# zjkang/Relation-DETR

Hardware: AMD Instinct MI355X
Metric: images/sec @ 800×1333, 300 queries, R50 4-level; achieved HBM GB/s (higher is better)
Workload: dtype bf16; 1 GPU; relation_detr_resnet50_800_1333 transformer stack from feature pyramids: 6 encoder layers (MSDA self-attn, S=22323, 4 levels) + two-stage top-k + 6 decoder layers (relation-biased self-attn + MSDA cross-attn + box refinement) + top-300 detections; backbone/neck excluded; batch_per_gpu=4, global_batch=4, queries=900, levels=4, launch=hipGraph replay, streams=2, gemm_tuning=False, parallelism=image-parallel x1

## Files before the change

### relation_detr_amd/csrc/linear.hip

```cpp
#include <cstdlib>

#include "launch.h"

namespace rdetr {

typedef __bf16 ln_bf16x8 __attribute__((ext_vector_type(8)));

constexpr int kLinK = 256;
constexpr int kLinThreads = 512;
constexpr int kLinRows = 32;

template <int NT, bool RELU>
__global__ __launch_bounds__(kLinThreads) void linear_k256_kernel(const uint16_t *__restrict__ x, long long ldx,
                                                                  const uint16_t *__restrict__ w, const uint16_t *__restrict__ bias,
                                                                  long long M, int N, uint16_t *__restrict__ out, long long ldo, int dbg,
                                                                  const unsigned char *__restrict__ row_mask, int hm_S)
{
    extern __shared__ __attribute__((aligned(16))) unsigned char lin_lds[];
    u32x4 *wl = reinterpret_cast<u32x4 *>(lin_lds);
    float *bl = reinterpret_cast<float *>(lin_lds + NT * 8 * 64 * 16);
    const int tid = threadIdx.x, lane = tid & 63, wave = tid >> 6;
    const int col = lane & 15, g = lane >> 4;
    const int n0 = blockIdx.y * (NT * 16);

    {
        constexpr int kPer = NT * 16 * 32 / kLinThreads;
        u32x4 piece[kPer];
#pragma unroll
        for (int i = 0; i < kPer; ++i) {
            const int idx = i * kLinThreads + tid, c = idx >> 5, p = idx & 31;
            piece[i] = n0 + c < N ? *reinterpret_cast<const u32x4 *>(w + (size_t)(n0 + c) * kLinK + 8 * p) : u32x4{0u, 0u, 0u, 0u};
        }
#pragma unroll
        for (int i = 0; i < kPer; ++i) {
            const int idx = i * kLinThreads + tid, c = idx >> 5, p = idx & 31;
            const int t = 2 * (c >> 5) + ((c >> 2) & 1), m = 4 * ((c >> 3) & 3) + (c & 3);
            wl[(t * 8 + (p >> 2)) * 64 + 16 * (p & 3) + m] = piece[i];
        }
    }
    for (int i = tid; i < NT * 16; i += kLinThreads) bl[i] = (bias && n0 + i < N) ? bf16_bits_to_f32(bias[n0 + i]) : 0.f;
    __syncthreads();

    const long long nsteps = (M + kLinRows - 1) / kLinRows;
    constexpr int kWaves = kLinThreads / 64;
    const long long stride = (long long)gridDim.x * kWaves;
    long long step = (long long)blockIdx.x * kWaves + wave;

    u32x4 xc[2][8], xn[2][8];
    auto load_rows = [&](long long st, u32x4 (&dst)[2][8]) {
#pragma unroll
        for (int cb = 0; cb < 2; ++cb) {
            const long long row = st * kLinRows + cb * 16 + col;
            const uint16_t *p = x + row * ldx + 8 * g;
#pragma unroll
            for (int s = 0; s < 8; ++s)
                dst[cb][s] = (st < nsteps && row < M) ? *reinterpret_cast<const u32x4 *>(p + 32 * s) : u32x4{0u, 0u, 0u, 0u};
        }
    };
    load_rows(step, xc);
    for (; step < nsteps; step += stride) {
        load_rows(step + stride, xn);
        const long long row_a = step * kLinRows + col, row_b = row_a + 16;
        uint16_t *oa = out + row_a * ldo + n0 + 8 * g, *ob = out + row_b * ldo + n0 + 8 * g;
        bool zero_a = false, zero_b = false;
        if (hm_S) {
            const unsigned ia = (unsigned)row_a / (unsigned)hm_S, ib = (unsigned)row_b / (unsigned)hm_S;
            oa = out + ((long long)ia * 8 * hm_S + (row_a - (long long)ia * hm_S)) * 32 + 8 * g;
            ob = out + ((long long)ib * 8 * hm_S + (row_b - (long long)ib * hm_S)) * 32 + 8 * g;
            if (row_mask) {
                zero_a = row_a < M && row_mask[row_a] != 0;
                zero_b = row_b < M && row_mask[row_b] != 0;
            }
        }
#pragma unroll
        for (int u = 0; u < NT / 2; ++u) {
            f32x4 acc[2][2];
#pragma unroll
            for (int e = 0; e < 2; ++e) {
                const f32x4 b4 = *reinterpret_cast<const f32x4 *>(bl + 32 * u + 8 * g + 4 * e);
                acc[e][0] = b4;
                acc[e][1] = b4;
            }
            if (!(dbg & 2))
#pragma unroll
            for (int s = 0; s < 8; ++s) {
#pragma unroll
                for (int e = 0; e < 2; ++e) {
                    const ln_bf16x8 a = __builtin_bit_cast(ln_bf16x8, wl[((2 * u + e) * 8 + s) * 64 + lane]);
                    acc[e][0] = __builtin_amdgcn_mfma_f32_16x16x32_bf16(a, __builtin_bit_cast(ln_bf16x8, xc[0][s]), acc[e][0], 0, 0, 0);
                    acc[e][1] = __builtin_amdgcn_mfma_f32_16x16x32_bf16(a, __builtin_bit_cast(ln_bf16x8, xc[1][s]), acc[e][1], 0, 0, 0);
                }
            }
            if (n0 + 32 * u + 8 * g < N) {
#pragma unroll
                for (int cb = 0; cb < 2; ++cb) {
                    f32x4 lo = acc[0][cb], hi = acc[1][cb];
                    if (RELU) {
                        lo.x = fmaxf(lo.x, 0.f); lo.y = fmaxf(lo.y, 0.f); lo.z = fmaxf(lo.z, 0.f); lo.w = fmaxf(lo.w, 0.f);
                        hi.x = fmaxf(hi.x, 0.f); hi.y = fmaxf(hi.y, 0.f); hi.z = fmaxf(hi.z, 0.f); hi.w = fmaxf(hi.w, 0.f);
                    }
                    u32x4 pk;
                    pk.x = f32_to_bf16_bits(lo.x) | (f32_to_bf16_bits(lo.y) << 16);
                    pk.y = f32_to_bf16_bits(lo.z) | (f32_to_bf16_bits(lo.w) << 16);
                    pk.z = f32_to_bf16_bits(hi.x) | (f32_to_bf16_bits(hi.y) << 16);
                    pk.w = f32_to_bf16_bits(hi.z) | (f32_to_bf16_bits(hi.w) << 16);
                    if ((cb ? zero_b : zero_a)) pk = u32x4{0u, 0u, 0u, 0u};
                    const long long col_off = hm_S ? (long long)u * hm_S * 32 : 32 * u;
                    if ((cb ? row_b : row_a) < M && !((dbg & 1) && pk.x != 0x12345u)) *reinterpret_cast<u32x4 *>((cb ? ob : oa) + col_off) = pk;
                }
            }
            __builtin_amdgcn_sched_barrier(0);
        }
#pragma unroll
        for (int cb = 0; cb < 2; ++cb)
#pragma unroll
            for (int s = 0; s < 8; ++s) xc[cb][s] = xn[cb][s];
    }
}

template <int NT, bool RELU>
static int linear_launch(const uint16_t *x, long long ldx, const uint16_t *w, const uint16_t *bias, long long M, int N,
                         uint16_t *out, long long ldo, int chunks, hipStream_t st, const unsigned char *row_mask = nullptr, int hm_S = 0)
{
    constexpr int lds = NT * 8 * 64 * 16 + NT * 16 * 4;
    if (const int s = ensure_dynamic_lds<linear_k256_kernel<NT, RELU>>(lds)) return s;
    const long long steps = (M + kLinRows - 1) / kLinRows;
    long long gx = (steps + kLinThreads / 64 - 1) / (kLinThreads / 64);
    const long long cap = kCus / chunks > 0 ? kCus / chunks : 1;
    if (gx > cap) gx = cap;
    hipLaunchKernelGGL((linear_k256_kernel<NT, RELU>), dim3((unsigned)gx, (unsigned)chunks), dim3(kLinThreads), (size_t)lds, st, x, ldx, w, bias, M, N, out,
                       ldo, 0, row_mask, hm_S);
    return launch_status();
}


constexpr int kLnlThreads = 512;
constexpr int kLnlWaves = kLnlThreads / 64;

__global__ __launch_bounds__(256) void linear_pack_kernel(const uint16_t *__restrict__ w, u32x4 *__restrict__ packed)
{
    const int idx = blockIdx.x * 256 + threadIdx.x;
    if (idx >= 16 * 8 * 64) return;
    const int t = idx >> 9, s = (idx >> 6) & 7, l = idx & 63, m = l & 15, kb = l >> 4;
    const int n = 32 * (t >> 1) + 8 * (m >> 2) + 4 * (t & 1) + (m & 3);
    packed[idx] = *reinterpret_cast<const u32x4 *>(w + (size_t)n * kLinK + 32 * s + 8 * kb);
}

__global__ __launch_bounds__(kLnlThreads) void linear_ln_k256_kernel(const uint16_t *__restrict__ x, long long ldx,
                                                                     const uint16_t *__restrict__ packed,
                                                                     const uint16_t *__restrict__ bias,
                                                                     const uint16_t *__restrict__ res, long long ldr,
                                                                     const uint16_t *__restrict__ gamma,
                                                                     const uint16_t *__restrict__ beta, float eps, long long M,
                                                                     uint16_t *__restrict__ out, long long ldo)
{
    extern __shared__ __attribute__((aligned(16))) unsigned char lin_lds[];
    const u32x4 *wl = reinterpret_cast<const u32x4 *>(lin_lds);
    float *bl = reinterpret_cast<float *>(lin_lds + 16 * 8 * 64 * 16);
    const int tid = threadIdx.x, lane = tid & 63, wave = __builtin_amdgcn_readfirstlane(tid >> 6);
    const int col = lane & 15, g = lane >> 4;
    {
        const unsigned lane_off = (unsigned)lane * 16u;
#pragma unroll 1
        for (int i = 0; i < 128 / kLnlWaves; ++i) {
            const int f = wave * (128 / kLnlWaves) + i;
            const unsigned m0v = (unsigned)f * 1024u;
            const unsigned char *src = reinterpret_cast<const unsigned char *>(packed) + f * 1024;
            asm volatile("s_mov_b32 m0, %0\n\ts_nop 0\n\tglobal_load_lds_dwordx4 %1, %2" : : "s"(m0v), "v"(lane_off), "s"(src) : "memory", "m0");
        }
    }
    if (tid < 256) {
        bl[tid] = bias ? bf16_bits_to_f32(bias[tid]) : 0.f;
        bl[256 + tid] = bf16_bits_to_f32(gamma[tid]);
        bl[512 + tid] = bf16_bits_to_f32(beta[tid]);
    }
    const long long nsteps = (M + kLinRows - 1) / kLinRows;
    long long step = (long long)blockIdx.x * kLnlWaves + wave;
    const long long stride = (long long)gridDim.x * kLnlWaves;
    asm volatile("s_waitcnt vmcnt(0)" ::: "memory");
    __syncthreads();
    for (; step < nsteps; step += stride) {
        const long long row_a = step * kLinRows + col, row_b = row_a + 16;
        u32x4 xc[2][8];
#pragma unroll
        for (int s = 0; s < 8; ++s) {
            xc[0][s] = row_a < M ? *reinterpret_cast<const u32x4 *>(x + row_a * ldx + 32 * s + 8 * g) : u32x4{0u, 0u, 0u, 0u};
            xc[1][s] = row_b < M ? *reinterpret_cast<const u32x4 *>(x + row_b * ldx + 32 * s + 8 * g) : u32x4{0u, 0u, 0u, 0u};
        }
        f32x4 acc[16][2];
        {
            auto frag = [&](int i) -> u32x4 { return wl[((i & 15) * 8 + (i >> 4)) * 64 + lane]; };
            const f32x4 zero4 = {0.f, 0.f, 0.f, 0.f};
            u32x4 ring[3];
            ring[0] = frag(0);
            ring[1] = frag(1);
#pragma unroll
            for (int i = 0; i < 128; ++i) {
                if (i + 2 < 128) ring[(i + 2) % 3] = frag(i + 2);
                __builtin_amdgcn_sched_barrier(0);
                const int s = i >> 4, t = i & 15;
                const ln_bf16x8 a = __builtin_bit_cast(ln_bf16x8, ring[i % 3]);
                acc[t][0] = __builtin_amdgcn_mfma_f32_16x16x32_bf16(a, __builtin_bit_cast(ln_bf16x8, xc[0][s]), s ? acc[t][0] : zero4, 0, 0, 0);
                acc[t][1] = __builtin_amdgcn_mfma_f32_16x16x32_bf16(a, __builtin_bit_cast(ln_bf16x8, xc[1][s]), s ? acc[t][1] : zero4, 0, 0, 0);
                __builtin_amdgcn_sched_barrier(0);
            }
        }
#pragma unroll
        for (int cb = 0; cb < 2; ++cb) {
            const long long row = cb ? row_b : row_a;
            const bool ok = row < M;
            float sum = 0.f;
#pragma unroll
            for (int u = 0; u < 8; ++u) {
                const u32x4 r = ok ? *reinterpret_cast<const u32x4 *>(res + row * ldr + 32 * u + 8 * g) : u32x4{0u, 0u, 0u, 0u};
                f32x4 &lo = acc[2 * u][cb], &hi = acc[2 * u + 1][cb];
                lo += *reinterpret_cast<const f32x4 *>(bl + 32 * u + 8 * g);
                hi += *reinterpret_cast<const f32x4 *>(bl + 32 * u + 8 * g + 4);
                const unsigned p0 = pack_bf16x2(lo.x, lo.y), p1 = pack_bf16x2(lo.z, lo.w), p2 = pack_bf16x2(hi.x, hi.y), p3 = pack_bf16x2(hi.z, hi.w);
                lo.x = __builtin_bit_cast(float, p0 << 16) + __builtin_bit_cast(float, r.x << 16);
                lo.y = __builtin_bit_cast(float, p0 & 0xffff0000u) + __builtin_bit_cast(float, r.x & 0xffff0000u);
                lo.z = __builtin_bit_cast(float, p1 << 16) + __builtin_bit_cast(float, r.y << 16);
                lo.w = __builtin_bit_cast(float, p1 & 0xffff0000u) + __builtin_bit_cast(float, r.y & 0xffff0000u);
                hi.x = __builtin_bit_cast(float, p2 << 16) + __builtin_bit_cast(float, r.z << 16);
                hi.y = __builtin_bit_cast(float, p2 & 0xffff0000u) + __builtin_bit_cast(float, r.z & 0xffff0000u);
                hi.z = __builtin_bit_cast(float, p3 << 16) + __builtin_bit_cast(float, r.w << 16);
                hi.w = __builtin_bit_cast(float, p3 & 0xffff0000u) + __builtin_bit_cast(float, r.w & 0xffff0000u);
                sum += ((lo.x + lo.y) + (lo.z + lo.w)) + ((hi.x + hi.y) + (hi.z + hi.w));
            }
            sum += __shfl_xor(sum, 16, 64);
            sum += __shfl_xor(sum, 32, 64);
            const float mean = sum * (1.0f / 256.0f);
            float sq = 0.f;
#pragma unroll
            for (int u = 0; u < 8; ++u) {
                f32x4 &lo = acc[2 * u][cb], &hi = acc[2 * u + 1][cb];
                lo.x -= mean; lo.y -= mean; lo.z -= mean; lo.w -= mean;
                hi.x -= mean; hi.y -= mean; hi.z -= mean; hi.w -= mean;
                sq += ((lo.x * lo.x + lo.y * lo.y) + (lo.z * lo.z + lo.w * lo.w)) + ((hi.x * hi.x + hi.y * hi.y) + (hi.z * hi.z + hi.w * hi.w));
            }
            sq += __shfl_xor(sq, 16, 64);
            sq += __shfl_xor(sq, 32, 64);
            const float rstd = 1.0f / sqrtf(sq * (1.0f / 256.0f) + eps);
#pragma unroll
            for (int u = 0; u < 8; ++u) {
                const f32x4 lo = acc[2 * u][cb], hi = acc[2 * u + 1][cb];
                const float *gp = bl + 256 + 32 * u + 8 * g, *bp = bl + 512 + 32 * u + 8 * g;
                const f32x4 g0 = *reinterpret_cast<const f32x4 *>(gp), g1 = *reinterpret_cast<const f32x4 *>(gp + 4);
                const f32x4 c0 = *reinterpret_cast<const f32x4 *>(bp), c1 = *reinterpret_cast<const f32x4 *>(bp + 4);
                u32x4 pk;
                pk.x = pack_bf16x2(lo.x * rstd * g0.x + c0.x, lo.y * rstd * g0.y + c0.y);
                pk.y = pack_bf16x2(lo.z * rstd * g0.z + c0.z, lo.w * rstd * g0.w + c0.w);
                pk.z = pack_bf16x2(hi.x * rstd * g1.x + c1.x, hi.y * rstd * g1.y + c1.y);
                pk.w = pack_bf16x2(hi.z * rstd * g1.z + c1.z, hi.w * rstd * g1.w + c1.w);
                if (ok) *reinterpret_cast<u32x4 *>(out + row * ldo + 32 * u + 8 * g) = pk;
            }
        }
    }
}

}

using namespace rdetr;

extern "C" int rdetr_linear_k256_bf16(const uint16_t *x, long long ldx, const uint16_t *w, const uint16_t *bias, long long M,
                                      int N, int relu, uint16_t *out, long long ldo, void *stream)
{
    if (M < 0 || N <= 0) return RDETR_ERR_INVALID_ARG;
    if (const int s = rows_status({{x, ldx, kLinK, 2}, {out, ldo, N, 2}})) return s;
    if (N & 31) return RDETR_ERR_UNSUPPORTED;
    if (M == 0) return RDETR_OK;
    if (!x || !w || !out) return RDETR_ERR_INVALID_ARG;
    if (!aligned_to(w, 16)) return RDETR_ERR_UNSUPPORTED;
    hipStream_t st = static_cast<hipStream_t>(stream);
    if (N % 256 == 0 || N < 192 || (N % 192 != 0)) {
        const int chunks = (N + 255) / 256;
        return relu ? linear_launch<16, true>(x, ldx, w, bias, M, N, out, ldo, chunks, st)
                    : linear_launch<16, false>(x, ldx, w, bias, M, N, out, ldo, chunks, st);
    }
    const int chunks = N / 192;
    return relu ? linear_launch<12, true>(x, ldx, w, bias, M, N, out, ldo, chunks, st)
                : linear_launch<12, false>(x, ldx, w, bias, M, N, out, ldo, chunks, st);
}

extern "C" int rdetr_linear_k256_hm_bf16(const uint16_t *x, long long ldx, const uint16_t *w, const uint16_t *bias,
                                         const uint8_t *row_mask, int B, int S, uint16_t *out_hm, void *stream)
{
    if (B < 0 || S < 0) return RDETR_ERR_INVALID_ARG;
    if (const int s = rows_status({{x, ldx, kLinK, 2}})) return s;
    if (B == 0 || S == 0) return RDETR_OK;
    if ((long long)B * S >= (1ll << 31)) return RDETR_ERR_UNSUPPORTED;
    if (!x || !w || !out_hm) return RDETR_ERR_INVALID_ARG;
    if (!all_aligned(16, w, out_hm)) return RDETR_ERR_UNSUPPORTED;
    return linear_launch<16, false>(x, ldx, w, bias, (long long)B * S, 256, out_hm, 256, 1, static_cast<hipStream_t>(stream), row_mask, S);
}

extern "C" int rdetr_linear_pack_k256_bf16(const uint16_t *w, uint16_t *packed, void *stream)
{
    if (!w || !packed) return RDETR_ERR_INVALID_ARG;
    if (!all_aligned(16, w, packed)) return RDETR_ERR_UNSUPPORTED;
    hipLaunchKernelGGL(linear_pack_kernel, dim3(32), dim3(256), 0, static_cast<hipStream_t>(stream), w, reinterpret_cast<u32x4 *>(packed));
    return launch_status();
}

extern "C" int rdetr_linear_ln_k256_bf16(const uint16_t *x, long long ldx, const uint16_t *packed, const uint16_t *bias,
                                         const uint16_t *residual, long long ldr, const uint16_t *gamma, const uint16_t *beta,
                                         float eps, long long M, uint16_t *out, long long ldo, void *stream)
{
    if (M < 0) return RDETR_ERR_INVALID_ARG;
    if (const int s = rows_status({{x, ldx, kLinK, 2}, {residual, ldr, kLinK, 2}, {out, ldo, kLinK, 2}})) return s;
    if (M == 0) return RDETR_OK;
    if (!x || !packed || !residual || !gamma || !beta || !out) return RDETR_ERR_INVALID_ARG;
    if (!aligned_to(packed, 16)) return RDETR_ERR_UNSUPPORTED;
    constexpr int lds = 16 * 8 * 64 * 16 + 3 * 256 * 4;
    if (const int s = ensure_dynamic_lds<linear_ln_k256_kernel>(lds)) return s;
    const long long steps = (M + kLinRows - 1) / kLinRows;
    long long gx = (steps + kLnlWaves - 1) / kLnlWaves;
    if (gx > kCus) gx = kCus;
    hipLaunchKernelGGL(linear_ln_k256_kernel, dim3((unsigned)gx), dim3(kLnlThreads), (size_t)lds, static_cast<hipStream_t>(stream), x,
                       ldx, packed, bias, residual, ldr, gamma, beta, eps, M, out, ldo);
    return launch_status();
}
```

### relation_detr_amd/csrc/proj.hip

```cpp
#include <type_traits>

#include "launch.h"

namespace rdetr {

namespace {

typedef __bf16 pj_bf16x8 __attribute__((ext_vector_type(8)));

constexpr int kPjHalf = 8 * 8 * 64 * 16;
constexpr int kPjLdsBias = kPjHalf;
constexpr int kPjLdsBytes = kPjLdsBias + (256 + 512) * 4;

template <int CB, int THREADS, int QCOLS>
__global__ __launch_bounds__(THREADS) void encoder_proj_k256_kernel(
    const uint16_t *__restrict__ x, long long ldx, const uint16_t *__restrict__ xq, long long ldq, const uint16_t *__restrict__ pwv,
    const uint16_t *__restrict__ bv, const uint16_t *__restrict__ pwq, const uint16_t *__restrict__ bq,
    const unsigned char *__restrict__ row_mask, int S, long long M, uint16_t *__restrict__ out_hm, uint16_t *__restrict__ out_q)
{
    constexpr int kMaxFrags = CB == 2 ? 8 : 8;
    extern __shared__ __attribute__((aligned(16))) unsigned char pj_lds[];
    const u32x4 *wl = reinterpret_cast<const u32x4 *>(pj_lds);
    float *bl = reinterpret_cast<float *>(pj_lds + kPjLdsBias);
    const int tid = threadIdx.x, lane = tid & 63, wave = __builtin_amdgcn_readfirstlane(tid >> 6);
    const int nwaves = (int)(blockDim.x >> 6);
    const int col = lane & 15, g = lane >> 4;

    u32x4 stg[kMaxFrags];
    auto fetch = [&](const uint16_t *packed, int h) {
#pragma unroll
        for (int i = 0; i < kMaxFrags; ++i) {
            const int f = wave + i * nwaves;
            if (f < 64) stg[i] = reinterpret_cast<const u32x4 *>(packed)[((size_t)h * kPjHalf + (size_t)f * 1024) / 16 + lane];
        }
        __builtin_amdgcn_sched_barrier(0);
    };
    auto commit = [&]() {
        __syncthreads();
        u32x4 *dst = reinterpret_cast<u32x4 *>(pj_lds);
#pragma unroll
        for (int i = 0; i < kMaxFrags; ++i) {
            const int f = wave + i * nwaves;
            if (f < 64) dst[f * 64 + lane] = stg[i];
        }
        __syncthreads();
    };

    fetch(pwv, 0);
    for (int i = tid; i < 256; i += (int)blockDim.x) bl[i] = bv ? bf16_bits_to_f32(bv[i]) : 0.f;
    for (int i = tid; i < 512; i += (int)blockDim.x) bl[256 + i] = (bq && i < QCOLS) ? bf16_bits_to_f32(bq[i]) : 0.f;

    const long long row0 = ((long long)blockIdx.x * nwaves + wave) * (16 * CB) + col;
    u32x4 xr[CB][8], qr[CB][8];
    bool rok[CB], zero[CB];
    uint16_t *ohm[CB], *oq[CB];
#pragma unroll
    for (int cb = 0; cb < CB; ++cb) {
        const long long row = row0 + 16 * cb;
        rok[cb] = row < M;
        const long long r = rok[cb] ? row : 0;
#pragma unroll
        for (int s = 0; s < 8; ++s) {
            xr[cb][s] = rok[cb] ? *reinterpret_cast<const u32x4 *>(x + r * ldx + 32 * s + 8 * g) : u32x4{0u, 0u, 0u, 0u};
            qr[cb][s] = rok[cb] ? *reinterpret_cast<const u32x4 *>(xq + r * ldq + 32 * s + 8 * g) : u32x4{0u, 0u, 0u, 0u};
        }
        zero[cb] = rok[cb] && row_mask && row_mask[r] != 0;
        const long long img = r / S, pos = r - img * S;
        ohm[cb] = out_hm + ((img * 8) * (long long)S + pos) * 32 + 8 * g;
        oq[cb] = out_q + r * QCOLS + 8 * g;
    }

    auto mm = [&](const u32x4 &a, const u32x4 &bq_, const f32x4 &c) {
        return __builtin_amdgcn_mfma_f32_16x16x32_bf16(__builtin_bit_cast(pj_bf16x8, a), __builtin_bit_cast(pj_bf16x8, bq_), c, 0, 0, 0);
    };
    auto block = [&](const u32x4 (&xin)[CB][8], f32x4 (&acc)[4][2][CB], auto nfrags) {
        constexpr int kFrags = decltype(nfrags)::value, kAhead = 3;
        u32x4 ring[4];
        auto frag = [&](int f) { return wl[(((2 * (f >> 4) + (f & 1)) * 8 + ((f >> 1) & 7)) * 64) + lane]; };
#pragma unroll
        for (int f = 0; f < kAhead; ++f) ring[f & 3] = frag(f);
        const f32x4 zero4 = {0.f, 0.f, 0.f, 0.f};
#pragma unroll
        for (int f = 0; f < kFrags; ++f) {
            if (f + kAhead < kFrags) ring[(f + kAhead) & 3] = frag(f + kAhead);
            __builtin_amdgcn_sched_barrier(0);
#pragma unroll
            for (int cb = 0; cb < CB; ++cb)
                acc[f >> 4][f & 1][cb] = mm(ring[f & 3], xin[cb][(f >> 1) & 7], ((f >> 1) & 7) ? acc[f >> 4][f & 1][cb] : zero4);
            __builtin_amdgcn_sched_barrier(0);
        }
    };
    auto packed_out = [&](const f32x4 (&acc)[4][2][CB], const float *bias, int uu, int cb) {
        const f32x4 lo = acc[uu][0][cb] + *reinterpret_cast<const f32x4 *>(bias + 32 * uu + 8 * g);
        const f32x4 hi = acc[uu][1][cb] + *reinterpret_cast<const f32x4 *>(bias + 32 * uu + 8 * g + 4);
        return u32x4{pack_bf16x2(lo.x, lo.y), pack_bf16x2(lo.z, lo.w), pack_bf16x2(hi.x, hi.y), pack_bf16x2(hi.z, hi.w)};
    };

    constexpr int kBlocks = 2 + (QCOLS + 127) / 128;
    constexpr int kLastUnits = (QCOLS - 128 * (kBlocks - 3)) / 32;
    f32x4 acc[4][2][CB];
    commit();
#pragma unroll
    for (int p = 0; p < kBlocks; ++p) {
        if (p == 0) fetch(pwv, 1);
        else if (p < kBlocks - 1) fetch(pwq, p - 1);
        if (p < 2) {
            block(xr, acc, std::integral_constant<int, 64>{});
#pragma unroll
            for (int cb = 0; cb < CB; ++cb)
                if (rok[cb]) {
#pragma unroll
                    for (int uu = 0; uu < 4; ++uu) {
                        const u32x4 v = zero[cb] ? u32x4{0u, 0u, 0u, 0u} : packed_out(acc, bl + 128 * p, uu, cb);
                        *reinterpret_cast<u32x4 *>(ohm[cb] + (long long)(4 * p + uu) * S * 32) = v;
                    }
                }
        } else {
            constexpr int kUnitsOf[2] = {4, kLastUnits};
            const int units = kUnitsOf[p == kBlocks - 1];
            if (p == kBlocks - 1) block(qr, acc, std::integral_constant<int, 16 * kLastUnits>{});
            else block(qr, acc, std::integral_constant<int, 64>{});
#pragma unroll
            for (int cb = 0; cb < CB; ++cb)
                if (rok[cb]) {
#pragma unroll
                    for (int uu = 0; uu < 4; ++uu)
                        if (uu < units)
                            *reinterpret_cast<u32x4 *>(oq[cb] + 128 * (p - 2) + 32 * uu) = packed_out(acc, bl + 256 + 128 * (p - 2), uu, cb);
                }
        }
        if (p < kBlocks - 1) commit();
    }
}

}

}

using namespace rdetr;

extern "C" int rdetr_encoder_proj_k256_bf16(const uint16_t *x, long long ldx, const uint16_t *xq, long long ldq, const uint16_t *pwv,
                                            const uint16_t *bv, const uint16_t *pwq, const uint16_t *bq, const uint8_t *row_mask, int B, int S,
                                            int q_cols, uint16_t *out_hm, uint16_t *out_q, void *stream)
{
    if (B < 0 || S < 0) return RDETR_ERR_INVALID_ARG;
    if (const int s = rows_status({{x, ldx, 256, 2}, {xq, ldq, 256, 2}})) return s;
    if (q_cols != 384 && q_cols != 480) return RDETR_ERR_UNSUPPORTED;
    if (B == 0 || S == 0) return RDETR_OK;
    if (!x || !xq || !pwv || !pwq || !out_hm || !out_q) return RDETR_ERR_INVALID_ARG;
    if (!all_aligned(16, pwv, pwq, out_hm, out_q)) return RDETR_ERR_UNSUPPORTED;
    const long long M = (long long)B * S;
    const auto rounds = [&](long long rows) { return ((M + rows - 1) / rows + kCus - 1) / kCus; };
    long long best = 4 * rounds(256);
    int thin = 0;
#ifndef RDETR_PROJ_THIN
#define RDETR_PROJ_THIN 1
#endif
    if (RDETR_PROJ_THIN)
        for (int w = 12; w >= 9; --w) {
            const long long cost = 3 * rounds(16 * w);
            if (cost < best || (cost == best && thin)) {
                best = cost;
                thin = w;
            }
        }
    const long long tile_rows = thin ? 16 * thin : 256;
    const long long ntiles = (M + tile_rows - 1) / tile_rows;
    if (!grid_fits(ntiles)) return RDETR_ERR_UNSUPPORTED;
    hipStream_t st = static_cast<hipStream_t>(stream);
    if (ensure_dynamic_lds<encoder_proj_k256_kernel<2, 512, 384>>(kPjLdsBytes) || ensure_dynamic_lds<encoder_proj_k256_kernel<1, 768, 384>>(kPjLdsBytes) ||
        ensure_dynamic_lds<encoder_proj_k256_kernel<2, 512, 480>>(kPjLdsBytes) || ensure_dynamic_lds<encoder_proj_k256_kernel<1, 768, 480>>(kPjLdsBytes))
        return RDETR_ERR_LAUNCH;
    auto launch = [&](auto kernel, unsigned threads) {
        hipLaunchKernelGGL(kernel, dim3((unsigned)ntiles), dim3(threads), kPjLdsBytes, st, x, ldx, xq, ldq, pwv, bv, pwq, bq, row_mask, S, M,
                           out_hm, out_q);
    };
    if (q_cols == 384) {
        if (thin) launch(encoder_proj_k256_kernel<1, 768, 384>, 64u * (unsigned)thin);
        else launch(encoder_proj_k256_kernel<2, 512, 384>, 512u);
    } else {
        if (thin) launch(encoder_proj_k256_kernel<1, 768, 480>, 64u * (unsigned)thin);
        else launch(encoder_proj_k256_kernel<2, 512, 480>, 512u);
    }
    return launch_status();
}
```

Measured before the change: 1156 images/s.

## Defer query-row loads in encoder projection and add dev-only debug knobs to linear-LN

The encoder projection kernel no longer loads both the value rows and the query rows up front. It loads the value rows first, issues the bias and row-mask loads together, and defers the query-row loads until just after the first weight-block fetch, so those loads overlap the value-projection MFMAs and fewer registers stay live early. The bias writes into LDS now use one thread per element instead of strided loops. Separately, the linear+LayerNorm kernel gains a debug argument that can skip residual loads, the weight prefetch, the MFMAs or the stores; it is compiled to a constant zero outside RDETR_DEV builds. The reordering relies on sched_barrier placement, and out-of-range rows now read row 0 without predication, which may add a few redundant loads.

After: 1146 images/s. Within noise of the previous version (-0.8%).

```diff
diff --git a/relation_detr_amd/csrc/linear.hip b/relation_detr_amd/csrc/linear.hip
--- a/relation_detr_amd/csrc/linear.hip
+++ b/relation_detr_amd/csrc/linear.hip
@@ -152,8 +152,13 @@
                                                                      const uint16_t *__restrict__ res, long long ldr,
                                                                      const uint16_t *__restrict__ gamma,
                                                                      const uint16_t *__restrict__ beta, float eps, long long M,
-                                                                     uint16_t *__restrict__ out, long long ldo)
-{
+                                                                     uint16_t *__restrict__ out, long long ldo, int dbg_arg)
+{
+#ifdef RDETR_DEV
+    const int dbg = dbg_arg;
+#else
+    constexpr int dbg = 0;
+#endif
     extern __shared__ __attribute__((aligned(16))) unsigned char lin_lds[];
     const u32x4 *wl = reinterpret_cast<const u32x4 *>(lin_lds);
     float *bl = reinterpret_cast<float *>(lin_lds + 16 * 8 * 64 * 16);
@@ -161,6 +166,7 @@
     const int col = lane & 15, g = lane >> 4;
     {
         const unsigned lane_off = (unsigned)lane * 16u;
+        if (!(dbg & 4))
 #pragma unroll 1
         for (int i = 0; i < 128 / kLnlWaves; ++i) {
             const int f = wave * (128 / kLnlWaves) + i;
@@ -194,6 +200,10 @@
             u32x4 ring[3];
             ring[0] = frag(0);
             ring[1] = frag(1);
+            if (dbg & 2) {
+#pragma unroll
+                for (int t = 0; t < 16; ++t) acc[t][0] = acc[t][1] = zero4;
+            } else
 #pragma unroll
             for (int i = 0; i < 128; ++i) {
                 if (i + 2 < 128) ring[(i + 2) % 3] = frag(i + 2);
@@ -212,7 +222,7 @@
             float sum = 0.f;
 #pragma unroll
             for (int u = 0; u < 8; ++u) {
-                const u32x4 r = ok ? *reinterpret_cast<const u32x4 *>(res + row * ldr + 32 * u + 8 * g) : u32x4{0u, 0u, 0u, 0u};
+                const u32x4 r = ok && !(dbg & 1) ? *reinterpret_cast<const u32x4 *>(res + row * ldr + 32 * u + 8 * g) : u32x4{0u, 0u, 0u, 0u};
                 f32x4 &lo = acc[2 * u][cb], &hi = acc[2 * u + 1][cb];
                 lo += *reinterpret_cast<const f32x4 *>(bl + 32 * u + 8 * g);
                 hi += *reinterpret_cast<const f32x4 *>(bl + 32 * u + 8 * g + 4);
@@ -252,7 +262,7 @@
                 pk.y = pack_bf16x2(lo.z * rstd * g0.z + c0.z, lo.w * rstd * g0.w + c0.w);
                 pk.z = pack_bf16x2(hi.x * rstd * g1.x + c1.x, hi.y * rstd * g1.y + c1.y);
                 pk.w = pack_bf16x2(hi.z * rstd * g1.z + c1.z, hi.w * rstd * g1.w + c1.w);
-                if (ok) *reinterpret_cast<u32x4 *>(out + row * ldo + 32 * u + 8 * g) = pk;
+                if (ok && !((dbg & 8) && pk.x != 0x12345u)) *reinterpret_cast<u32x4 *>(out + row * ldo + 32 * u + 8 * g) = pk;
             }
         }
     }
@@ -302,6 +312,14 @@
     return launch_status();
 }
 
+#ifdef RDETR_DEV
+static int g_lnl_dbg = 0;
+extern "C" void rdetr_dev_set_linear_ln_dbg(int v) { g_lnl_dbg = v; }
+#define RDETR_LNL_DBG g_lnl_dbg
+#else
+#define RDETR_LNL_DBG 0
+#endif
+
 extern "C" int rdetr_linear_ln_k256_bf16(const uint16_t *x, long long ldx, const uint16_t *packed, const uint16_t *bias,
                                          const uint16_t *residual, long long ldr, const uint16_t *gamma, const uint16_t *beta,
                                          float eps, long long M, uint16_t *out, long long ldo, void *stream)
@@ -317,6 +335,6 @@
     long long gx = (steps + kLnlWaves - 1) / kLnlWaves;
     if (gx > kCus) gx = kCus;
     hipLaunchKernelGGL(linear_ln_k256_kernel, dim3((unsigned)gx), dim3(kLnlThreads), (size_t)lds, static_cast<hipStream_t>(stream), x,
-                       ldx, packed, bias, residual, ldr, gamma, beta, eps, M, out, ldo);
+                       ldx, packed, bias, residual, ldr, gamma, beta, eps, M, out, ldo, RDETR_LNL_DBG);
     return launch_status();
 }
diff --git a/relation_detr_amd/csrc/proj.hip b/relation_detr_amd/csrc/proj.hip
--- a/relation_detr_amd/csrc/proj.hip
+++ b/relation_detr_amd/csrc/proj.hip
@@ -47,9 +47,6 @@
     };
 
     fetch(pwv, 0);
-    for (int i = tid; i < 256; i += (int)blockDim.x) bl[i] = bv ? bf16_bits_to_f32(bv[i]) : 0.f;
-    for (int i = tid; i < 512; i += (int)blockDim.x) bl[256 + i] = (bq && i < QCOLS) ? bf16_bits_to_f32(bq[i]) : 0.f;
-
     const long long row0 = ((long long)blockIdx.x * nwaves + wave) * (16 * CB) + col;
     u32x4 xr[CB][8], qr[CB][8];
     bool rok[CB], zero[CB];
@@ -60,16 +57,38 @@
         rok[cb] = row < M;
         const long long r = rok[cb] ? row : 0;
 #pragma unroll
-        for (int s = 0; s < 8; ++s) {
-            xr[cb][s] = rok[cb] ? *reinterpret_cast<const u32x4 *>(x + r * ldx + 32 * s + 8 * g) : u32x4{0u, 0u, 0u, 0u};
-            qr[cb][s] = rok[cb] ? *reinterpret_cast<const u32x4 *>(xq + r * ldq + 32 * s + 8 * g) : u32x4{0u, 0u, 0u, 0u};
-        }
-        zero[cb] = rok[cb] && row_mask && row_mask[r] != 0;
+        for (int s = 0; s < 8; ++s) xr[cb][s] = rok[cb] ? *reinterpret_cast<const u32x4 *>(x + r * ldx + 32 * s + 8 * g) : u32x4{0u, 0u, 0u, 0u};
+    }
+    __builtin_amdgcn_sched_barrier(0);
+    const unsigned vraw = (bv ? bv : pwv)[tid < 256 ? tid : 0], qraw = (bq ? bq : pwv)[tid < QCOLS ? tid : 0];
+    unsigned char mraw[CB];
+#pragma unroll
+    for (int cb = 0; cb < CB; ++cb)
+        mraw[cb] = (row_mask ? row_mask : reinterpret_cast<const unsigned char *>(pwv))[row_mask && rok[cb] ? row0 + 16 * cb : 0];
+    __builtin_amdgcn_sched_barrier(0);
+    if (tid < 256) bl[tid] = bv ? bf16_bits_to_f32(vraw) : 0.f;
+    if (tid < 512) bl[256 + tid] = (bq && tid < QCOLS) ? bf16_bits_to_f32(qraw) : 0.f;
+#pragma unroll
+    for (int cb = 0; cb < CB; ++cb) {
+        const long long row = row0 + 16 * cb;
+        const long long r = rok[cb] ? row : 0;
+        unsigned zf = rok[cb] && row_mask && mraw[cb] != 0;
+        asm volatile("" : "+v"(zf));
+        zero[cb] = zf != 0;
         const long long img = r / S, pos = r - img * S;
         ohm[cb] = out_hm + ((img * 8) * (long long)S + pos) * 32 + 8 * g;
         oq[cb] = out_q + r * QCOLS + 8 * g;
     }
 
+    auto load_q = [&]() {
+#pragma unroll
+        for (int cb = 0; cb < CB; ++cb) {
+            const long long r = rok[cb] ? row0 + 16 * cb : 0;
+#pragma unroll
+            for (int s = 0; s < 8; ++s) qr[cb][s] = *reinterpret_cast<const u32x4 *>(xq + r * ldq + 32 * s + 8 * g);
+        }
+        __builtin_amdgcn_sched_barrier(0);
+    };
     auto mm = [&](const u32x4 &a, const u32x4 &bq_, const f32x4 &c) {
         return __builtin_amdgcn_mfma_f32_16x16x32_bf16(__builtin_bit_cast(pj_bf16x8, a), __builtin_bit_cast(pj_bf16x8, bq_), c, 0, 0, 0);
     };
@@ -102,7 +121,10 @@
     commit();
 #pragma unroll
     for (int p = 0; p < kBlocks; ++p) {
-        if (p == 0) fetch(pwv, 1);
+        if (p == 0) {
+            fetch(pwv, 1);
+            load_q();
+        }
         else if (p < kBlocks - 1) fetch(pwq, p - 1);
         if (p < 2) {
             block(xr, acc, std::integral_constant<int, 64>{});
```
